# galatolofederico/clip-glass

Hardware: AMD Instinct MI355X
Metric: candidate latents scored/sec (GAN→CLIP fitness), StyleGAN2_ffhq_d pop=64 (higher is better)
Workload: dtype f16; 1 GPU; StyleGAN2_ffhq_d: StyleGAN2 config-f 1024px G+D + CLIP ViT-B/32, pop=64 per GPU, batch_size=4, n_obj=2; pop_per_gpu=64, global_pop=64, batch_size=4, parallelism=population-shard x1, device=AMD Radeon Graphics (gfx950:sramecc+:xnack-), 256 CUs, hbm_gib=288

## Files before the change

clip_glass_amd/csrc/conv_down.hip:

```cpp
#include "common.h"
#include "kernels.h"
#include <stdio.h>
#include <stdlib.h>

namespace {
constexpr int TH = 4, NT = 64, CIN = 32, VP = 65;
constexpr int V_BYTES = 9 * VP * 64;
constexpr int W_BYTES = 9 * NT * 64;
constexpr int EM_BYTES = 9 * 4 * 64;
constexpr int OFF_W = V_BYTES, OFF_EM = OFF_W + W_BYTES, OFF_C = OFF_EM + EM_BYTES, OFF_WS = OFF_C + NT * 4;
constexpr int LDS_BYTES = OFF_WS + NT * 64;

__device__ __forceinline__ int vaddr(int row, int col, int cg) {
    return row * (VP * 64) + (((col & ~3) | ((col + (col >> 2)) & 3)) << 6) + (cg << 4);
}
__device__ __forceinline__ int aaddr(int row, int slot, int lc) { return row * (VP * 64) + (slot << 6) + ((lc ^ ((slot >> 2) & 3)) << 4); }
__device__ __forceinline__ int waddr(int row, int lc) { return (row << 6) + ((lc ^ ((row >> 2) & 3)) << 4); }
__device__ __forceinline__ h8 fir4(h8 a, h8 b, h8 c, h8 d) {
    return (a + d) * (half_t)0.125f + (b + c) * (half_t)0.375f;
}
__device__ __forceinline__ int opaque(int v) { asm volatile("" : "+v"(v)); return v; }
__device__ __forceinline__ int uni(int v) { return __builtin_amdgcn_readfirstlane(v); }
struct RSet { h8 a[12]; h8 e[4]; h8 s[2]; int b, ty0, tx0, valid; };
}

struct DownParams {
    const half_t* h;
    const half_t* xs;
    const half_t* w1;
    const half_t* ws;
    const float* b1;
    half_t* y;
    int B, R;
};

__global__ __launch_bounds__(256, 2) void conv_down_kernel(DownParams p, int tiles_x, int tiles_y, int n_tiles, int per_block) {
    extern __shared__ __attribute__((aligned(16))) char smem[];
    char* Vs = smem;
    char* Ws = smem + OFF_W;
    float* Cb = (float*)(smem + OFF_C);
    const int tpi = tiles_x * tiles_y;
    const int R = p.R, Ro = R >> 1;
    const int first = blockIdx.x * per_block;
    const int last = min(first + per_block, n_tiles);
    if (first >= last) return;
    const h8 zero = {0, 0, 0, 0, 0, 0, 0, 0};

    int nx_it = first, nx_b, nx_ty, nx_tx;
    {
        nx_b = uni(first / tpi);
        const int trem = first - nx_b * tpi;
        nx_tx = uni(trem / tiles_y);
        nx_ty = uni(trem - nx_tx * tiles_y);
    }
    const half_t* is_img = nullptr;
    int is_oy = 0, is_rs = 0;
    auto issue_begin = [&](RSet& Rg) {
        Rg.valid = nx_it < last;
        Rg.b = nx_b; Rg.ty0 = nx_ty * TH; Rg.tx0 = nx_tx * 32;
        is_img = p.h + (long long)Rg.b * R * R * CIN;
        is_oy = 2 * Rg.ty0 - 2;
        is_rs = R * CIN;
        if (nx_it + 1 < last) {
            ++nx_it;
            if (++nx_ty == tiles_y) { nx_ty = 0; if (++nx_tx == tiles_x) { nx_tx = 0; ++nx_b; } }
        } else {
            nx_it = last;
        }
    };
    auto issue_rows = [&](RSet& Rg, int k0) {
        const int t = opaque(threadIdx.x), cg = t & 3, cs = t >> 2;
        const int xo = min(max(2 * Rg.tx0 - 2 + cs, 0), R - 1) * CIN + cg * 8;
#pragma unroll
        for (int k = 0; k < 6; ++k) {
            const int iy = min(max(is_oy + k0 + k, 0), R - 1);
            Rg.a[k0 + k] = *(const h8*)(is_img + iy * is_rs + xo);
        }
    };
    auto issue_rest = [&](RSet& Rg) {
        const int t = opaque(threadIdx.x), cg = t & 3;
        const int er = min(t >> 4, 8);
        const int exo = min(max(2 * Rg.tx0 - 2 + 64 + ((t >> 2) & 3), 0), R - 1) * CIN + cg * 8;
#pragma unroll
        for (int k = 0; k < 4; ++k) Rg.e[k] = *(const h8*)(is_img + min(max(is_oy + er + k, 0), R - 1) * is_rs + exo);
        const int lr = t & 31, kh = (t >> 5) & 1, wave = t >> 6;
        const half_t* xp = p.xs + (((long long)Rg.b * Ro + Rg.ty0 + wave) * Ro + Rg.tx0 + lr) * CIN + kh * 8;
        Rg.s[0] = *(const h8*)xp;
        Rg.s[1] = *(const h8*)(xp + 16);
    };
    auto issue = [&](RSet& Rg) {
        issue_begin(Rg);
        issue_rows(Rg, 0);
        issue_rows(Rg, 6);
        issue_rest(Rg);
    };

    {
        const int t = threadIdx.x;
#pragma unroll
        for (int k = 0; k < 9; ++k) {
            const int v = k * 256 + t, row = v >> 2;
            const int lc = (v & 3) ^ ((row >> 2) & 3);
            *(h8*)(Ws + v * 16) = *(const h8*)(p.w1 + (long long)row * CIN + lc * 8);
        }
        const int row = t >> 2, lc = (t & 3) ^ ((row >> 2) & 3);
        const h8 wsv = *(const h8*)(p.ws + (long long)row * CIN + lc * 8);
        h8 wss;
#pragma unroll
        for (int q = 0; q < 8; ++q) wss[q] = (half_t)((float)wsv[q] * 0.70710678118654752440f);
        *(h8*)(smem + OFF_WS + t * 16) = wss;
        if (t < NT) Cb[t] = p.b1[t];
    }

    auto step = [&](int it, RSet& Rg) {
        const int b = Rg.b, ty0 = Rg.ty0, tx0 = Rg.tx0, valid = Rg.valid;
        const int oy = 2 * ty0 - 2, ox = 2 * tx0 - 2;
        __syncthreads();
        {
            const int t = opaque(threadIdx.x), cg = t & 3, cs = t >> 2;
            const bool border = oy < 0 || ox < 0 || oy + 12 > R || ox + 68 > R;
            if (border) {
                const bool colok = (unsigned)(ox + cs) < (unsigned)R;
#pragma unroll
                for (int k = 0; k < 12; ++k) Rg.a[k] = (colok && (unsigned)(oy + k) < (unsigned)R) ? Rg.a[k] : zero;
                const int er = t >> 4;
                const bool ecok = (unsigned)(ox + 64 + ((t >> 2) & 3)) < (unsigned)R;
#pragma unroll
                for (int k = 0; k < 4; ++k) Rg.e[k] = (ecok && (unsigned)(oy + er + k) < (unsigned)R) ? Rg.e[k] : zero;
            }
#pragma unroll
            for (int r = 0; r < 9; ++r) *(h8*)(Vs + vaddr(r, cs, cg)) = fir4(Rg.a[r], Rg.a[r + 1], Rg.a[r + 2], Rg.a[r + 3]);
            if (t < 144) *(h8*)(smem + OFF_EM + t * 16) = fir4(Rg.e[0], Rg.e[1], Rg.e[2], Rg.e[3]);
        }
        const h8 xs0 = Rg.s[0], xs1 = Rg.s[1];
        issue_begin(Rg);
        issue_rows(Rg, 0);
        __syncthreads();
        {
            const int t = opaque(threadIdx.x), lane = t & 63, wave = uni(t >> 6);
            const int j = lane >> 2, cgl = lane & 3;
            auto hrow = [&](int rr) {
                h8 v[8];
#pragma unroll
                for (int k = 0; k < 4; ++k) v[k] = *(const h8*)(Vs + vaddr(rr, 4 * j + k, cgl));
                v[7] = zero;
                if (j < 15) {
#pragma unroll
                    for (int k = 4; k < 7; ++k) v[k] = *(const h8*)(Vs + vaddr(rr, 4 * j + k, cgl));
                } else {
#pragma unroll
                    for (int k = 0; k < 4; ++k) v[4 + k] = *(const h8*)(smem + OFF_EM + ((rr * 4 + k) * 4 + cgl) * 16);
                }
                h8 o[5];
#pragma unroll
                for (int i = 0; i < 4; ++i) o[i] = fir4(v[i], v[i + 1], v[i + 2], v[i + 3]);
                o[4] = fir4(v[4], v[5], v[6], v[7]);
                __builtin_amdgcn_wave_barrier();
#pragma unroll
                for (int i = 0; i < 4; ++i) {
                    const int c = 4 * j + i;
                    const int slot = (c & 1) ? 33 + (c >> 1) : (c >> 1);
                    *(h8*)(Vs + aaddr(rr, slot, cgl)) = o[i];
                }
                if (j == 15) *(h8*)(Vs + aaddr(rr, 32, cgl)) = o[4];
                __builtin_amdgcn_wave_barrier();
            };
            hrow(wave);
            __builtin_amdgcn_sched_barrier(0);
            issue_rows(Rg, 6);
            hrow(wave + 4);
            __builtin_amdgcn_sched_barrier(0);
            issue_rest(Rg);
            if (wave == 0) hrow(8);
        }
        __syncthreads();
        const int tm = opaque(threadIdx.x), lr = tm & 31, kh = (tm >> 5) & 1, wave = uni(tm >> 6);
        f16x acc[2];
#pragma unroll
        for (int j = 0; j < 2; ++j)
#pragma unroll
            for (int q = 0; q < 16; ++q) acc[j][q] = 0.f;
#pragma unroll
        for (int ky = 0; ky < 3; ++ky)
#pragma unroll
            for (int kx = 0; kx < 3; ++kx)
#pragma unroll
                for (int kk = 0; kk < 2; ++kk) {
                    const int lc = kk * 2 + kh;
                    const h8 xf = *(const h8*)(Vs + aaddr(2 * wave + ky, (kx == 1 ? 33 : (kx >> 1)) + lr, lc));
#pragma unroll
                    for (int j = 0; j < 2; ++j) {
                        const h8 wf = *(const h8*)(Ws + waddr((ky * 3 + kx) * NT + j * 32 + lr, lc));
                        acc[j] = mfma32(wf, xf, acc[j]);
                    }
                    if (kk && kx == 2) __builtin_amdgcn_sched_barrier(0);
                }
#pragma unroll
        for (int j = 0; j < 2; ++j)
#pragma unroll
            for (int g = 0; g < 4; ++g) {
                const f4 bb = *(const f4*)(Cb + j * 32 + 8 * g + 4 * kh);
#pragma unroll
                for (int q = 0; q < 4; ++q) {
                    const float v = acc[j][g * 4 + q] + bb[q];
                    acc[j][g * 4 + q] = fmaxf(v, 0.2f * v);
                }
            }
#pragma unroll
        for (int kk = 0; kk < 2; ++kk)
#pragma unroll
            for (int j = 0; j < 2; ++j) {
                const h8 wf = *(const h8*)(smem + OFF_WS + waddr(j * 32 + lr, kk * 2 + kh));
                acc[j] = mfma32(wf, kk ? xs1 : xs0, acc[j]);
            }
        const int lane = tm & 63;
        char* Os = Vs + (2 * wave + 1) * (VP * 64);
        __builtin_amdgcn_wave_barrier();
#pragma unroll
        for (int j = 0; j < 2; ++j)
#pragma unroll
            for (int g = 0; g < 4; ++g) {
                h4 out;
#pragma unroll
                for (int q = 0; q < 4; ++q) out[q] = (half_t)acc[j][g * 4 + q];
                *(h4*)(Os + lr * 128 + (((j * 4 + g) ^ (lr & 7)) << 4) + kh * 8) = out;
            }
        __builtin_amdgcn_wave_barrier();
        if (valid) {
            half_t* yrow = p.y + (((long long)b * Ro + ty0 + wave) * Ro + tx0) * NT;
#pragma unroll
            for (int k = 0; k < NT / 16; ++k) {
                const int v = lane + 64 * k;
                const int pix = v >> 3, chv = v & 7;
                *(h8*)(yrow + (long long)pix * NT + chv * 8) = *(const h8*)(Os + pix * 128 + ((chv ^ (pix & 7)) << 4));
            }
        }
    };

    RSet r0, r1;
    issue(r0);
    issue(r1);
    for (int it = first; it < last; it += 2) {
        step(it, r0);
        step(it + 1, r1);
    }
}

bool conv_down_supported(int R, int Cin, int Cout) {
    return glass_lds_fits(LDS_BYTES) && R % 64 == 0 && R >= 64 && Cin == CIN && Cout == NT && (long long)R * R * Cin < (1LL << 31);
}

const char* launch_conv_down(const half_t* h, const half_t* xs, const half_t* w1, const half_t* ws, const float* b1, half_t* y,
                             int B, int R, int Cin, int Cout, hipStream_t st) {
    if (!conv_down_supported(R, Cin, Cout)) return nullptr;
    DownParams p;
    p.h = h; p.xs = xs; p.w1 = w1; p.ws = ws; p.b1 = b1; p.y = y; p.B = B; p.R = R;
    const int Ro = R / 2, tiles_x = Ro / 32, tiles_y = Ro / TH;
    const long long tiles = (long long)B * tiles_x * tiles_y;
    if (tiles >= (1LL << 30)) return nullptr;
    static DevOnce once;
    once.run([&] { (void)hipFuncSetAttribute((const void*)conv_down_kernel, hipFuncAttributeMaxDynamicSharedMemorySize, LDS_BYTES); });
    const int slots = glass_cu_count() * 2;
    const int per_block = (int)((tiles + slots - 1) / slots);
    const int grid = (int)((tiles + per_block - 1) / per_block);
    hipLaunchKernelGGL(conv_down_kernel, dim3(grid), dim3(256), LDS_BYTES, st, p, tiles_x, tiles_y, (int)tiles, per_block);
    return "conv_down_kernel";
}
```

clip_glass_amd/csrc/kernels.h:

```cpp
#pragma once
#include "common.h"

#include <string>
#include <vector>

const char* launch_conv_direct(const ConvParams& p, hipStream_t st);
const char* launch_gemm_direct(const GemmParams& p, hipStream_t st);
const char* launch_conv_tiled(const ConvParams& p, hipStream_t st);
const char* launch_gemm_tiled(const GemmParams& p, hipStream_t st);
const char* launch_conv_stream(const ConvParams& p, hipStream_t st);
const char* launch_conv_gemm(const ConvParams& p, half_t* ws_a, long long cap_a, float* ws_c, long long cap_c, hipStream_t st);
bool conv_stream_applies(const ConvParams& p);
const char* launch_conv_glds(const ConvParams& p, hipStream_t st);
const char* launch_conv_wreg(const ConvParams& p, hipStream_t st);
bool conv_wreg_supported(int Cin, int Cout, int H, int W);
const char* launch_conv_s2(const ConvParams& p, hipStream_t st, bool force = false);
const char* launch_conv_down(const half_t* h, const half_t* xs, const half_t* w1, const half_t* ws, const float* b1, half_t* y,
                             int B, int R, int Cin, int Cout, hipStream_t st);
bool conv_down_supported(int R, int Cin, int Cout);
const char* launch_dblock0(const float* rgb_y, const float* rgb_w, const float* rgb_b, const half_t* w0, const float* b0, const half_t* w1,
                           const half_t* ws, const float* b1, half_t* y, int B, int R, int Cin, int Cout, hipStream_t st, int y_planar8 = 0);
bool dblock0_supported(int R, int Cin, int Cout);
const char* launch_upconv_fused(const ConvParams& p, hipStream_t st);

void launch_pixelnorm(const float* z, float* out, int P, int L, float eps, hipStream_t st);
void launch_dense01_finish(const float* part, int S, long long slab, const float* bias0, const float* w1, const float* b1, float* out, int P, int N,
                           hipStream_t st);
void launch_dense_splitk(const float* x, int ldx, int P, int K, const float* wt, int N, const float* bias, float* out, int ldo,
                         int mode, hipStream_t st);
void launch_dense(const float* x, int ldx, int P, int K, const float* wt, int N, const float* bias,
                  float* out, int ldo, int in_sq, int mode, const float* eps_row, int eps_stride,
                  hipStream_t st);
bool launch_mapping_fused(const float* z, float* out, int P, int L, float eps, const float* const* wt, const float* const* b, int n_layers,
                          hipStream_t st);
struct DenseDesc {
    const float* x; int ldx; int K; const float* wt; int N; const float* bias; float* out; int ldo;
    const float* eps_row; int eps_stride;
};
void launch_dense_multi(const DenseDesc* d_desc, int n_desc, int max_N, int P, int in_sq, int mode, hipStream_t st);
void launch_style_norm(float* s, int ld, int P, int n_layers, const int* d_off, const int* d_len,
                       float* smax, float* eps_row, float eps, hipStream_t st);
void launch_modulate_weights(const half_t* w, long long elems, int Cin, int Cout, const float* sn, int sn_stride,
                              const float* dscale, int ds_stride, int P, half_t* wm, hipStream_t st);
void launch_noise(float* out, int n_mb, int hw, uint32_t layer, uint32_t mb0, uint32_t generation,
                  uint64_t seed, hipStream_t st);

void launch_trgb_tables(const float* wrgb, const float* sn, int sn_stride, const float* smax, int smax_stride, int B, int NT,
                        half_t* tab, hipStream_t st);
void launch_trgb_finish(const float* part, int ntn, int B, int R, const float* bias, const float* yprev, float* yout, hipStream_t st);
bool launch_torgb(const half_t* x, int B, int H, int W, int C, const float* wrgb, const float* bias,
                  const float* sn, int sn_stride, const float* smax, int smax_stride,
                  const float* yprev, float* yout, hipStream_t st);
void launch_finalize_image(const float* y, float* img, long long n, hipStream_t st);
void launch_resize_patches(const float* y, int B, int R, int clip_res, int ps, int ld, half_t* patches,
                           hipStream_t st);
#define GLASS_RESIZE_MAX_TAPS 32
#define PREPROCESS_TY 8
#define PREPROCESS_RB 8
#define PREPROCESS_MAX_R 1024
struct ResizeTaps {
    std::vector<int> start, count;
    std::vector<float> taps;
    std::vector<float> table;
    int max_count = 0, nr = 0, ts = 0;
    size_t lds_bytes = 0;
};
struct ResizeTapsDev {
    const float* table = nullptr;
    int n4 = 0, ts = 0;
    size_t lds_bytes = 0;
};
bool build_resize_taps(int R, int S, int mode, ResizeTaps& t, std::string& why);
void launch_preprocess_patches(const float* y, int B, int R, int clip_res, int ps, int ld, int resize_mode, int normalize,
                               const ResizeTapsDev& t, half_t* patches, hipStream_t st);
void launch_fromrgb(const float* y, int B, int R, int Cout, const float* w, const float* bias,
                    half_t* out, hipStream_t st);
void launch_blur_pad2(const half_t* x, int B, int H, int W, int C, half_t* out, hipStream_t st, int planar32 = 0);
bool blur_pad2_planar32_ok(int C);
void launch_blur_down(const half_t* x, int B, int H, int W, int C, half_t* out, hipStream_t st);
void launch_mbstd(const half_t* x, int B, int hw, int C, int Cpad, int batch_size, int group, float eps,
                  half_t* out, hipStream_t st);

void launch_embed_lnpre(const float* patch_emb, const float* cls, const float* pos, const float* g,
                        const float* b, int P, int T, int D, float* x, hipStream_t st);
void launch_embed_text(const int* tokens, const float* tok_emb, const float* pos, int n_rows, int ctx, int D, float* x,
                       hipStream_t st);
void launch_layernorm(const float* x, long long row_stride, int M, int D, const float* g, const float* b,
                      half_t* out16, float* out32, hipStream_t st);
void launch_layernorm_rows(const float* x, const int* rows, int M, int D, const float* g, const float* b, float* out32, hipStream_t st);
void launch_attention(const half_t* qkv, int n_img, int L, int heads, int hd, int causal, half_t* out,
                      hipStream_t st);
void launch_cosine(const float* feat, const float* target, int P, int D, float* sim, hipStream_t st);
void launch_assemble_F(const float* sim, const float* dis, int P, int n_obj, float* F, hipStream_t st);

void launch_bg_cond(const float* x, int P, int L, int zd, int nc, const float* et, float* cond, hipStream_t st);
void launch_bg_bn_tables(float* tab, int P, int C, const float* inv_std, const float* mean, const float* prebias,
                         hipStream_t st);
void launch_bg_to_half(const float* x, half_t* y, long long n, hipStream_t st);
const char* launch_bg_attn_split(const half_t* T, int B, int H, int W, int c8, int c2, half_t* theta, half_t* phi, half_t* gT,
                                 hipStream_t st);
void launch_bg_softmax(const float* S, long long rows, int n, half_t* Pm, hipStream_t st);
void launch_bg_rgb_tanh(const half_t* x, int B, long long hw, int C, float* y, hipStream_t st);

struct BgTailParams {
    const half_t* h;
    const half_t* x0;
    const half_t* w3;
    const float* b3;
    const float* tab;
    int bnf_off, ctot;
    const half_t* rgb_w;
    int cpad;
    const float* rgb_b;
    float* y;
    int B, R;
};
bool bg_tail_supported(int R, int mid, int cout, int cin, int up, int cpad);
bool launch_bg_tail(const BgTailParams& p, hipStream_t st);
void launch_gpt2_embed(const int* tok, const float* wte, const float* wpe, int rows, int L, int pos0, int D, float* x,
                       hipStream_t st);
void launch_gemm_f32(const float* A, const float* W, const float* bias, float* out, int M, int N, int K, int lda, int ldo,
                     int mode, hipStream_t st, float* part = nullptr, size_t part_elems = 0, bool prefill = false);
bool gemm_f32_step_supported(int M, int K, int lda, bool ln_fused);
int launch_gemm_f32_step(const float* A, const float* W, const float* bias, float* out, int M, int N, int K, int lda, int ldo, int mode,
                         hipStream_t st, float* part, size_t part_elems, const float* stats, const float* lng, const float* lnb);
bool gpt2_head_supported(int M, int N, int K, int lda);
bool launch_gpt2_head_tail(const float* A, const float* W, int M, int N, int K, int lda, const float* stats_in, const float* lng, const float* lnb,
                           float* pairs, int* gen, int* state, const float* wte, const float* wpe, float* x, float* stats_out, hipStream_t st);
bool launch_gpt2_head(const float* A, const float* W, int M, int N, int K, int lda, const float* stats, const float* lng, const float* lnb,
                      float* logits, float* pairs, int* out, const int* step_dev, hipStream_t st);
void launch_gpt2_reduce(const float* part, int S, const float* bias, float* out, int M, int N, int ldo, int mode, hipStream_t st);
void launch_gpt2_finalize(const float* part, int S, const float* bias, float* x, int M, int D, float* stats, hipStream_t st);
#define GPT2_ATTENTION_LDS_MAX (160 * 1024)
size_t gpt2_attention_lds_bytes(int nd, int ns);
void launch_gpt2_attention(const float* qkv, float* kc, float* vc, int P, int nd, int past, int Tmax, int heads,
                           float* out, hipStream_t st, const int* past_dev = nullptr);
void launch_gpt2_attention_step(const float* qkv, const float* part, int S, const float* bias, float* kc, float* vc, int P, int Tmax, int heads,
                                float* out, hipStream_t st, const int* past_dev);
void launch_argmax(const float* logits, int rows, int N, int* out, hipStream_t st, const int* step_dev = nullptr, float* scratch = nullptr);
void launch_gpt2_embed_step(const int* gen, const int* state, int P, const float* wte, const float* wpe, int D, float* x, hipStream_t st,
                            float* stats = nullptr, bool partial_fmt = false);
bool gemm_f32_rowblk_supported(int M, int N, int K, int lda, bool ln_fused, bool stats_out);
bool launch_gemm_f32_rowblk(const float* A, const float* W, const float* bias, float* out, int M, int N, int K, int lda, int ldo, int mode,
                            hipStream_t st, const float* pst_in, int np_in, const float* lng, const float* lnb, float* pst_out);
void launch_gpt2_advance(int* state, hipStream_t st);
enum { GPT2_SP_SEED_LO, GPT2_SP_SEED_HI, GPT2_SP_GEN, GPT2_SP_ROW0, GPT2_SP_PURPOSE, GPT2_SP_TEMP, GPT2_SP_TOPK, GPT2_SP_STEP, GPT2_SP_WORDS };
#define GPT2_SAMPLE_TOPK_MAX 256
bool gpt2_sample_supported(int V);
void launch_gpt2_sample(const float* logits, int rows, int V, const int* sp, int* out, int* state, hipStream_t st);
bool launch_gpt2_head_sample(const float* A, const float* W, int M, int N, int K, int lda, const float* stats_in, const float* lng, const float* lnb,
                             float* logits, float* pairs, const int* sp, int* gen, int* state, bool tail, const float* wte, const float* wpe, float* x,
                             float* stats_out, hipStream_t st);
void launch_image_patches(const float* img, int n, int S, int ps, int ld, half_t* patches, hipStream_t st);
```

Measured before the change: 2204 candidates/s.

## Add fused downsample conv kernel for 64-to-128 channel discriminator blocks

Adds a new conv_down64 kernel for the StyleGAN2 discriminator downsampling block with 64 input and 128 output channels, selected automatically when Cin is 64. It fuses the FIR blur, the stride-2 3x3 conv through MFMA with register-resident weights, bias plus leaky ReLU, and the scaled 1x1 skip conv. It uses a persistent rolling row pipeline with prefetched registers and one 512-thread block per CU. Previously this shape fell back to a less fused path. The cost is heavy register and LDS use at occupancy 1.

Result: faster. 2253 candidates/s, median of 6 (+2.2%).

```diff
diff --git a/clip_glass_amd/csrc/conv_down.hip b/clip_glass_amd/csrc/conv_down.hip
--- a/clip_glass_amd/csrc/conv_down.hip
+++ b/clip_glass_amd/csrc/conv_down.hip
@@ -247,12 +247,14 @@
 }
 
 bool conv_down_supported(int R, int Cin, int Cout) {
+    if (Cin == 64) return conv_down64_supported(R, Cin, Cout);
     return glass_lds_fits(LDS_BYTES) && R % 64 == 0 && R >= 64 && Cin == CIN && Cout == NT && (long long)R * R * Cin < (1LL << 31);
 }
 
 const char* launch_conv_down(const half_t* h, const half_t* xs, const half_t* w1, const half_t* ws, const float* b1, half_t* y,
                              int B, int R, int Cin, int Cout, hipStream_t st) {
     if (!conv_down_supported(R, Cin, Cout)) return nullptr;
+    if (Cin == 64) return launch_conv_down64(h, xs, w1, ws, b1, y, B, R, Cin, Cout, st);
     DownParams p;
     p.h = h; p.xs = xs; p.w1 = w1; p.ws = ws; p.b1 = b1; p.y = y; p.B = B; p.R = R;
     const int Ro = R / 2, tiles_x = Ro / 32, tiles_y = Ro / TH;
diff --git a/clip_glass_amd/csrc/conv_down64.hip b/clip_glass_amd/csrc/conv_down64.hip
--- /dev/null
+++ b/clip_glass_amd/csrc/conv_down64.hip
@@ -0,0 +1,219 @@
+#include "common.h"
+#include "kernels.h"
+
+namespace {
+constexpr int TW = 29, CIN = 64, COUT = 128;
+constexpr int ROWB = 64 * 128;
+constexpr int V_BYTES = 4 * ROWB;
+constexpr int A_BYTES = 8 * ROWB;
+constexpr int XS_BYTES = 2 * 32 * 128;
+constexpr int O_BYTES = 2 * 32 * 256;
+constexpr int OFF_A = V_BYTES, OFF_XS = OFF_A + A_BYTES, OFF_O = OFF_XS + XS_BYTES, OFF_C = OFF_O + O_BYTES;
+constexpr int LDS_BYTES = OFF_C + COUT * 4;
+
+__device__ __forceinline__ int vaddr(int row, int col, int cg) { return row * ROWB + ((col ^ ((col >> 2) & 1)) << 7) + (cg << 4); }
+__device__ __forceinline__ int aaddr(int rslot, int slot, int lc) { return rslot * ROWB + (slot << 7) + ((lc ^ ((slot >> 1) & 7)) << 4); }
+__device__ __forceinline__ int oaddr(int row, int px, int c16) { return row * (32 * 256) + (px << 8) + ((c16 ^ (px & 15)) << 4); }
+__device__ __forceinline__ h8 fir4(h8 a, h8 b, h8 c, h8 d) {
+    const half_t q = (half_t)0.125f, t = (half_t)0.375f;
+    const h8 k125 = {q, q, q, q, q, q, q, q}, k375 = {t, t, t, t, t, t, t, t};
+    return __builtin_elementwise_fma(b + c, k375, (a + d) * k125);
+}
+__device__ __forceinline__ int opaque(int v) { asm volatile("" : "+v"(v)); return v; }
+__device__ __forceinline__ int uni(int v) { return __builtin_amdgcn_readfirstlane(v); }
+struct RSet { h8 a[4]; h8 x; int b, tx, s, valid; };
+}
+
+struct Down64Params {
+    const half_t* h;
+    const half_t* xs;
+    const half_t* w1;
+    const half_t* ws;
+    const float* b1;
+    half_t* y;
+    int B, R;
+};
+
+__global__ __launch_bounds__(512, 1) void conv_down64_kernel(Down64Params p, int tiles_x, int SY, int n_steps, int per_block) {
+    extern __shared__ __attribute__((aligned(16))) char smem[];
+    char* Vs = smem;
+    char* As = smem + OFF_A;
+    char* Xs = smem + OFF_XS;
+    char* Os = smem + OFF_O;
+    float* Cb = (float*)(smem + OFF_C);
+    const int R = p.R, Ro = R >> 1;
+    const int first = blockIdx.x * per_block;
+    const int last = min(first + per_block, n_steps);
+    if (first >= last) return;
+    const h8 zero = {0, 0, 0, 0, 0, 0, 0, 0};
+
+    int nx_left = last - first, nx_prime = 1, nx_b, nx_tx, nx_s;
+    {
+        const int per_img = tiles_x * SY;
+        nx_b = uni(first / per_img);
+        const int rem = first - nx_b * per_img;
+        nx_tx = uni(rem / SY);
+        nx_s = uni(rem - nx_tx * SY);
+    }
+    const int total = nx_left + 1 + (nx_s + nx_left - 1) / SY;
+
+    auto issue = [&](RSet& Rg) {
+        Rg.b = nx_b; Rg.tx = nx_tx;
+        if (nx_prime) {
+            Rg.s = nx_s - 1; Rg.valid = 0; nx_prime = 0;
+        } else {
+            Rg.s = nx_s; Rg.valid = nx_left > 0;
+            if (nx_left > 1) {
+                if (++nx_s == SY) { nx_s = 0; nx_prime = 1; if (++nx_tx == tiles_x) { nx_tx = 0; ++nx_b; } }
+            }
+            if (nx_left > 0) --nx_left;
+        }
+        const int t = opaque(threadIdx.x), cg = t & 7, cs = t >> 3;
+        const half_t* img = p.h + (long long)Rg.b * R * R * CIN;
+        const int xo = min(max(2 * TW * Rg.tx - 2 + cs, 0), R - 1) * CIN + cg * 8;
+#pragma unroll
+        for (int k = 0; k < 4; ++k) {
+            const int iy = min(max(4 * Rg.s + 2 + k, 0), R - 1);
+            Rg.a[k] = *(const h8*)(img + iy * (R * CIN) + xo);
+        }
+        const int v = min(t, 2 * TW * 8 - 1), row = v >= TW * 8, rem = v - row * (TW * 8);
+        const int yy = min(max(2 * Rg.s + row, 0), Ro - 1), xx = min(TW * Rg.tx + (rem >> 3), Ro - 1);
+        Rg.x = *(const h8*)(p.xs + (((long long)Rg.b * Ro + yy) * Ro + xx) * CIN + (rem & 7) * 8);
+    };
+
+    h8 Wm[9][4], Wk[4];
+    {
+        const int t = threadIdx.x, lr = t & 31, kh = (t >> 5) & 1, nb = (t >> 6) & 3;
+#pragma unroll
+        for (int tap = 0; tap < 9; ++tap)
+#pragma unroll
+            for (int kk = 0; kk < 4; ++kk) Wm[tap][kk] = *(const h8*)(p.w1 + ((tap * COUT + nb * 32 + lr) * CIN + kk * 16 + kh * 8));
+#pragma unroll
+        for (int kk = 0; kk < 4; ++kk) {
+            const h8 wv = *(const h8*)(p.ws + ((nb * 32 + lr) * CIN + kk * 16 + kh * 8));
+#pragma unroll
+            for (int q = 0; q < 8; ++q) Wk[kk][q] = (half_t)((float)wv[q] * 0.70710678118654752440f);
+        }
+        if (t < COUT) Cb[t] = p.b1[t];
+    }
+
+    h8 c0 = zero, c1 = zero, c2 = zero;
+
+    auto step = [&](RSet& Rg) {
+        const int b = Rg.b, tx = Rg.tx, s = Rg.s, valid = Rg.valid;
+        const int ox = 2 * TW * tx - 2, oy = 4 * s + 2;
+        __syncthreads();
+        {
+            const int t = opaque(threadIdx.x), cg = t & 7, cs = t >> 3;
+            const bool border = ox < 0 || ox + 64 > R || oy < 0 || oy + 4 > R;
+            if (border) {
+                const bool colok = (unsigned)(ox + cs) < (unsigned)R;
+#pragma unroll
+                for (int k = 0; k < 4; ++k) Rg.a[k] = (colok && (unsigned)(oy + k) < (unsigned)R) ? Rg.a[k] : zero;
+            }
+            *(h8*)(Vs + vaddr(0, cs, cg)) = fir4(c0, c1, c2, Rg.a[0]);
+            *(h8*)(Vs + vaddr(1, cs, cg)) = fir4(c1, c2, Rg.a[0], Rg.a[1]);
+            *(h8*)(Vs + vaddr(2, cs, cg)) = fir4(c2, Rg.a[0], Rg.a[1], Rg.a[2]);
+            *(h8*)(Vs + vaddr(3, cs, cg)) = fir4(Rg.a[0], Rg.a[1], Rg.a[2], Rg.a[3]);
+            c0 = Rg.a[1]; c1 = Rg.a[2]; c2 = Rg.a[3];
+            if (t < 2 * TW * 8) {
+                const int row = t >= TW * 8, rem = t - row * (TW * 8);
+                *(h8*)(Xs + aaddr(0, row * 32 + (rem >> 3), rem & 7)) = Rg.x;
+            }
+        }
+        issue(Rg);
+        __syncthreads();
+        {
+            const int t = opaque(threadIdx.x), lane = t & 63, wave = uni(t >> 6);
+            const int row = wave >> 1, j = (wave & 1) * 8 + (lane >> 3), cg = lane & 7;
+            if (j < 15) {
+                h8 v[7];
+#pragma unroll
+                for (int k = 0; k < 7; ++k) v[k] = *(const h8*)(Vs + vaddr(row, 4 * j + k, cg));
+                const int rslot = (4 * s + 1 + row) & 7;
+#pragma unroll
+                for (int i = 0; i < 4; ++i) {
+                    const int c = 4 * j + i;
+                    const int slot = (c & 1) ? 32 + (c >> 1) : (c >> 1);
+                    *(h8*)(As + aaddr(rslot, slot, cg)) = fir4(v[i], v[i + 1], v[i + 2], v[i + 3]);
+                }
+            }
+        }
+        __syncthreads();
+        const int tm = opaque(threadIdx.x), lr = tm & 31, kh = (tm >> 5) & 1, wave = uni(tm >> 6), r = wave >> 2, nb = wave & 3;
+        f16x acc;
+#pragma unroll
+        for (int q = 0; q < 16; ++q) acc[q] = 0.f;
+#pragma unroll
+        for (int ky = 0; ky < 3; ++ky) {
+            const int rslot = (4 * s + 2 * r + ky) & 7;
+#pragma unroll
+            for (int kx = 0; kx < 3; ++kx)
+#pragma unroll
+                for (int kk = 0; kk < 4; ++kk) {
+                    const h8 xf = *(const h8*)(As + aaddr(rslot, (kx == 1 ? 32 : (kx >> 1)) + lr, kk * 2 + kh));
+                    acc = mfma32(Wm[ky * 3 + kx][kk], xf, acc);
+                    if (kk == 3 && (kx & 1) == (ky & 1)) __builtin_amdgcn_sched_barrier(0);
+                }
+        }
+#pragma unroll
+        for (int g = 0; g < 4; ++g) {
+            const f4 bb = *(const f4*)(Cb + nb * 32 + 8 * g + 4 * kh);
+#pragma unroll
+            for (int q = 0; q < 4; ++q) {
+                const float v = acc[g * 4 + q] + bb[q];
+                acc[g * 4 + q] = fmaxf(v, 0.2f * v);
+            }
+        }
+#pragma unroll
+        for (int kk = 0; kk < 4; ++kk) acc = mfma32(Wk[kk], *(const h8*)(Xs + aaddr(0, r * 32 + lr, kk * 2 + kh)), acc);
+#pragma unroll
+        for (int g = 0; g < 4; ++g) {
+            h4 out;
+#pragma unroll
+            for (int q = 0; q < 4; ++q) out[q] = (half_t)acc[g * 4 + q];
+            *(h4*)(Os + oaddr(r, lr, nb * 4 + g) + kh * 8) = out;
+        }
+        __syncthreads();
+        if (valid) {
+            const int t = opaque(threadIdx.x);
+            const int npx = min(TW, Ro - TW * tx);
+#pragma unroll
+            for (int k = 0; k < 2; ++k) {
+                const int v = t + 512 * k;
+                const int row = v >= TW * 16, rem = v - row * (TW * 16), px = rem >> 4, ch = rem & 15;
+                if (v < 2 * TW * 16 && px < npx)
+                    *(h8*)(p.y + (((long long)b * Ro + 2 * s + row) * Ro + TW * tx + px) * COUT + ch * 8) = *(const h8*)(Os + oaddr(row, px, ch));
+            }
+        }
+    };
+
+    RSet r0, r1;
+    issue(r0);
+    issue(r1);
+    for (int it = 0; it < total; it += 2) {
+        step(r0);
+        step(r1);
+    }
+}
+
+bool conv_down64_supported(int R, int Cin, int Cout) {
+    return Cin == CIN && Cout == COUT && R >= 16 && R % 4 == 0 && (long long)R * R * Cin < (1LL << 31) && glass_lds_fits(LDS_BYTES);
+}
+
+const char* launch_conv_down64(const half_t* h, const half_t* xs, const half_t* w1, const half_t* ws, const float* b1, half_t* y,
+                               int B, int R, int Cin, int Cout, hipStream_t st) {
+    if (!conv_down64_supported(R, Cin, Cout)) return nullptr;
+    Down64Params p;
+    p.h = h; p.xs = xs; p.w1 = w1; p.ws = ws; p.b1 = b1; p.y = y; p.B = B; p.R = R;
+    const int Ro = R / 2, tiles_x = (Ro + TW - 1) / TW, SY = Ro / 2;
+    const long long steps = (long long)B * tiles_x * SY;
+    if (steps >= (1LL << 30)) return nullptr;
+    static DevOnce once;
+    once.run([&] { (void)hipFuncSetAttribute((const void*)conv_down64_kernel, hipFuncAttributeMaxDynamicSharedMemorySize, LDS_BYTES); });
+    const int slots = glass_cu_count();
+    const int per_block = (int)((steps + slots - 1) / slots);
+    const int grid = (int)((steps + per_block - 1) / per_block);
+    hipLaunchKernelGGL(conv_down64_kernel, dim3(grid), dim3(512), LDS_BYTES, st, p, tiles_x, SY, (int)steps, per_block);
+    return "conv_down64_kernel";
+}
diff --git a/clip_glass_amd/csrc/kernels.h b/clip_glass_amd/csrc/kernels.h
--- a/clip_glass_amd/csrc/kernels.h
+++ b/clip_glass_amd/csrc/kernels.h
@@ -18,6 +18,9 @@
 const char* launch_conv_down(const half_t* h, const half_t* xs, const half_t* w1, const half_t* ws, const float* b1, half_t* y,
                              int B, int R, int Cin, int Cout, hipStream_t st);
 bool conv_down_supported(int R, int Cin, int Cout);
+const char* launch_conv_down64(const half_t* h, const half_t* xs, const half_t* w1, const half_t* ws, const float* b1, half_t* y,
+                               int B, int R, int Cin, int Cout, hipStream_t st);
+bool conv_down64_supported(int R, int Cin, int Cout);
 const char* launch_dblock0(const float* rgb_y, const float* rgb_w, const float* rgb_b, const half_t* w0, const float* b0, const half_t* w1,
                            const half_t* ws, const float* b1, half_t* y, int B, int R, int Cin, int Cout, hipStream_t st, int y_planar8 = 0);
 bool dblock0_supported(int R, int Cin, int Cout);
```
